# apirrone/Open_Duck_Playground

Measured on AMD Instinct MI355X. Metric: env-steps/sec open_duck_mini_v2 flat_terrain @8192 envs; 1/2/4/8-GPU scaling, higher is better.
Workload: dtype f32

## Files before the change

include/odk.h:

```cpp
#ifndef ODK_H
#define ODK_H

#include <stdint.h>

#ifdef __cplusplus
extern "C" {
#endif

typedef struct odk_model odk_model;
typedef struct odk_batch odk_batch;

enum odk_status {
  ODK_OK = 0,
  ODK_ERR_INVALID = -1,
  ODK_ERR_UNSUPPORTED = -2,
  ODK_ERR_HIP = -3,
  ODK_ERR_NOMEM = -4
};

#define ODK_NOBS 101
#define ODK_NPRIV 212
#define ODK_NOBS_STANDING 85
#define ODK_NPRIV_STANDING 153
#define ODK_ENV_JOYSTICK 0
// ... 348 lines not shown
} odk_step_tail;
int odk_adam_clip_packed_tail(float* params_dev, const float* grads_dev, float* m_dev, float* v_dev, float* acc_dev, long long n, float lr, float b1,
                              float b2, float eps, float max_grad_norm, float* fwd_packed_dev, long long n_fwd, float* bwd_packed_dev, long long n_bwd,
                              const odk_weight_table* table, int norm_blocks, const odk_step_tail* tail , void* stream);

#define ODK_GAE_HEAD_SAMPLES 32
typedef struct odk_gae_head_args {
  const float *logits, *values, *raw_action, *old_log_prob, *reward, *termination, *truncation, *noise;
  const long long* row_idx;
  const int* cursor;
  float *dlogits, *dvalues, *losses, *loss_partials, *adv_out, *vs_out, *stats_out;
  int B, T, action_size, n_traj, normalize_advantage;
  float gae_lambda, discount, clipping_epsilon, entropy_cost, grad_scale;
} odk_gae_head_args;
int odk_ppo_gae_head(const odk_gae_head_args* args, void* stream);

int odk_col_moments(const float* x_dev, long long rows, int w, int slices, double* partial_dev, void* stream);
int odk_moments_update(const double* partial_dev, int slices, int w, long long rows, double* count_dev, float* mean_dev, float* summed_variance_dev,
                       float* std_dev, float std_min, float std_max, void* stream);

int odk_colsum_fold(const float* const* partial_dev, float* const* colsum_dev, const int* widths, const int* nblk, int count, void* stream);

int odk_gather_rows(const float* const* src_dev, float* const* dst_dev, const int* row_floats, const long long* direct_base, int nfields,
                    const long long* idx_dev, int nrows, long long src_rows, void* stream);

int odk_batch_timing(odk_batch* b, int enable, float* avg_ms, int* launches);

#ifdef __cplusplus
}
#endif
// ... 2 lines not shown
```

open_duck_playground_amd/csrc/odk_learner.hip:

```cpp
#include <hip/hip_runtime.h>
#include <algorithm>
#include <utility>
#include <vector>
#include <stdint.h>
#include <string.h>

#include <type_traits>

#include "../../include/odk.h"
#include "odk_host.h"
#include "odk_poison.h"

int odk_func_lds_attr_(const void* fn, int slot, int bytes);

namespace {

__device__ __forceinline__ float wave_sum(float v) {
#pragma unroll
  for (int o = 32; o >= 1; o >>= 1) v += __shfl_xor(v, o);
  return v;
}
__device__ __forceinline__ float row16_sum(float v) {
#pragma unroll
  for (int o = 8; o >= 1; o >>= 1) v += __shfl_xor(v, o);
  return v;
}
__device__ float block_sum(float v, float* sh) {
  v = wave_sum(v);
  const int w = threadIdx.x >> 6, nw = blockDim.x >> 6;
  __syncthreads();
  if ((threadIdx.x & 63) == 0) sh[w] = v;
  __syncthreads();
  float t = 0.0f;
  for (int i = 0; i < nw; i++) t += sh[i];
  return t;
}
__device__ __forceinline__ float softplus(float x) { return x > 20.0f ? x : log1pf(__expf(x)); }
__device__ __forceinline__ float sigmoid(float x) { return 1.0f / (1.0f + __expf(-x)); }

__device__ __forceinline__ float gae_step(float r, float v, float mask, float nt, float discount, float lambda_, float& acc, float& v_next, float& vs_next,
                                          float& vs_t) {
  const float dn = __fmul_rn(discount, nt);
  const float delta = __fmul_rn(__fsub_rn(__fmaf_rn(dn, v_next, r), v), mask);
  acc = __fmaf_rn(__fmul_rn(__fmul_rn(dn, mask), lambda_), acc, delta);
  vs_t = __fadd_rn(acc, v);
  const float a = __fmul_rn(__fsub_rn(__fmaf_rn(dn, vs_next, r), v), mask);
  v_next = v; vs_next = vs_t;
  return a;
}

__global__ void gae_kernel(const float* __restrict__ trunc, const float* __restrict__ term, const float* __restrict__ rew,
                           const float* __restrict__ val, const float* __restrict__ boot, float* __restrict__ vs,
                           float* __restrict__ adv, float* __restrict__ stats, int B, int T, float lambda_, float discount) {
  __shared__ float sh[16];
#ifdef ODK_POISON_LDS
  odk_poison_fill(sh, sizeof(sh) / 4);
  __syncthreads();
#endif
  float s = 0.0f;
  for (int b = threadIdx.x; b < B; b += blockDim.x) {
    const size_t o = (size_t)b * T;
    float acc = 0.0f, v_next = boot[b], vs_next = boot[b];
    for (int t = T - 1; t >= 0; t--) {
// ... 85 lines not shown
      s = __fadd_rn(s, a);
    }
  }
  __syncthreads();
  for (int i = threadIdx.x; i < N; i += blockDim.x) { adv[i] = s_r[i]; vs[i] = s_v[i]; }
  if (!stats) return;
  const float n = (float)B * (float)T;
  const float mean = block_sum(s, sh) / n;
  float q = 0.0f;
  for (int b = threadIdx.x; b < B; b += blockDim.x)
    for (int t = 0; t < T; t++) { const float d = s_r[b * T + t] - mean; q = __fmaf_rn(d, d, q); }
  const float var = block_sum(q, sh) / n;
  if (threadIdx.x == 0) { stats[0] = mean; stats[1] = 1.0f / (sqrtf(var) + 1e-8f); }
}

struct HeadOut { float dloc, dscale_raw, dbaseline, lp, lv, le; };
__device__ __forceinline__ HeadOut head_sample(bool on, float loc, float raw, float a, float z, float advn, float old_lp, float vs_s, float base_s, float inv_n,
                                               float eps, float entropy_cost, float grad_scale) {
  const float HALF_LOG_2PI = 0.91893853320467274f, LOG2 = 0.69314718055994531f;
  const float scale = softplus(raw) + 0.001f, inv_scale = 1.0f / scale, lscale = __logf(scale);
  const float u = (a - loc) * inv_scale;
  const float ldj_a = 2.0f * (LOG2 - a - softplus(-2.0f * a));
  const float lp_j = on ? (-0.5f * u * u - lscale - HALF_LOG_2PI - ldj_a) : 0.0f;
  const float x = loc + scale * z;
  const float ldj_x = 2.0f * (LOG2 - x - softplus(-2.0f * x));
  const float ent_j = on ? (0.5f + HALF_LOG_2PI + lscale + ldj_x) : 0.0f;
  const float logp = row16_sum(lp_j), ent = row16_sum(ent_j);
  const float rho = __expf(logp - old_lp);
  const float rc = fminf(fmaxf(rho, 1.0f - eps), 1.0f + eps);
  const float s1 = rho * advn, s2 = rc * advn;
  const bool inside = rho >= 1.0f - eps && rho <= 1.0f + eps;
  const float dmin_drho = (inside || s1 < s2) ? advn : 0.0f;
  const float dL_dlogp = -dmin_drho * rho * inv_n;
  const float verr = vs_s - base_s;
  const float th = tanhf(x);
  const float ce = -entropy_cost * inv_n;
  HeadOut o;
  o.dloc = grad_scale * (dL_dlogp * u * inv_scale + ce * (-2.0f * th));
  o.dscale_raw = grad_scale * (dL_dlogp * (u * u - 1.0f) * inv_scale + ce * (inv_scale - 2.0f * th * z)) * sigmoid(raw);
  o.dbaseline = grad_scale * (-0.5f * verr * inv_n);
  o.lp = -fminf(s1, s2) * inv_n; o.lv = 0.25f * verr * verr * inv_n; o.le = -entropy_cost * ent * inv_n;
  return o;
}

__global__ void ppo_head_kernel(const float* __restrict__ logits, const float* __restrict__ raw_action, const float* __restrict__ old_logp,
                                const float* __restrict__ adv, const float* __restrict__ stats, const float* __restrict__ vs,
                                const float* __restrict__ baseline, const float* __restrict__ noise, float* __restrict__ dlogits,
                                float* __restrict__ dbaseline, float* __restrict__ losses, int n, int A, float eps, float entropy_cost,
                                float grad_scale) {
  const int lane = threadIdx.x & 15;
  const int s = (blockIdx.x * blockDim.x + threadIdx.x) >> 4;
  const bool live = s < n, on = live && lane < A;
  const int sc = live ? s : n - 1;
  float loc = 0.f, raw = 0.f, a = 0.f, z = 0.f;
  if (on) { loc = logits[(size_t)sc * 2 * A + lane]; raw = logits[(size_t)sc * 2 * A + A + lane]; a = raw_action[(size_t)sc * A + lane]; z = noise[(size_t)sc * A + lane]; }
  float advn = adv[sc];
  if (stats) advn = (advn - stats[0]) * stats[1];
  const HeadOut h = head_sample(on, loc, raw, a, z, advn, old_logp[sc], vs[sc], baseline[sc], 1.0f / (float)n, eps, entropy_cost, grad_scale);
// ... 768 lines not shown
```

open_duck_playground_amd/csrc/odk_mlp.hip:

```cpp
#include <hip/hip_runtime.h>
#include <stdint.h>
#include <stdlib.h>
#include <string.h>

#include "../../include/odk.h"
#include "odk_host.h"
#include "odk_poison.h"

namespace {

typedef float f32x4 __attribute__((ext_vector_type(4)));

constexpr int H1 = ODK_MLP_H1, H2 = ODK_MLP_H2, H3 = ODK_MLP_H3;
constexpr int TM = ODK_MLP_TILE;
constexpr int CH = 128;
constexpr int KIN_MAX = ODK_MLP_MAX_IN, NOUT_MAX = 32;
constexpr int PC = CH + 4, P2 = H2 + 4, P3 = H3 + 4, P4 = NOUT_MAX + 4;
constexpr int PX_MAX = KIN_MAX + 4;
constexpr int SLACK = 64;
static_assert(TM == 16 && KIN_MAX % 16 == 0, "tile = one 16-row MFMA block, padded input width");
constexpr int F_X = 0, F_C = F_X + TM * PX_MAX, F_H2 = F_C + TM * PC, F_TOTAL = F_H2 + TM * P2 + SLACK;
static_assert(TM * P3 <= TM * PX_MAX, "layer-3 output must fit in the X region");
static_assert(3 * 2 * 4 * 64 <= TM * PC, "output-layer partial blocks must fit in the chunk region");
static_assert(F_TOTAL * 4 <= 40 * 1024, "four forward workgroups per CU");
constexpr int B_D4 = 0, B_D3 = B_D4 + TM * P4, B_D2 = B_D3 + TM * P3, B_TOTAL = B_D2 + TM * P2 + SLACK;

__host__ __device__ constexpr int pad16(int k) { return (k + 15) & ~15; }

struct Net {
  const float* x; const float* in_mean; const float* in_std; const float* wf[4]; const float* wb[4]; const float* b[4];
  float* h[3]; float* g[3]; float* out; float* xp;
  const float* dout; float* dz[3]; float* doutp; float* bias_partial[4];
  int n, n_in, n_out, tile0;
  const long long* row_idx; const int* cursor; const float* x_tail; int traj_len, n_main, n_traj;
};
struct Map { int R, rounds, rem, vin2, pin2, v3, costly, on; };
struct Args { Net net[2]; int nnets; long long* prof; long long* wgprof; Map map; };
__device__ __forceinline__ void map_block(const Args& a, int b, int& net, int& tile) {
  const Map& m = a.map;
  if (!m.on) { net = (a.nnets > 1 && b >= a.net[1].tile0) ? 1 : 0; tile = b - a.net[net].tile0; return; }
  const int k = b % m.R, r = b / m.R;
  bool costly; int idx;
  if (k >= m.rem) { const int s2 = (k - m.rem) * m.rounds + r; costly = s2 < m.vin2; idx = costly ? s2 : s2 - m.vin2; }
  else { const int c = r * m.rem + k; costly = c < m.v3; idx = costly ? m.vin2 + c : m.pin2 + (c - m.v3); }
  net = costly ? m.costly : 1 - m.costly; tile = idx;
}
#define ODK_WG_BEGIN() long long wg_t0 = 0, wg_c0 = 0; if (a.wgprof) { wg_t0 = wall_clock64(); wg_c0 = clock64(); }
#define ODK_WG_END() do { if (a.wgprof && threadIdx.x == 0) { long long* o = a.wgprof + 4 * blockIdx.x; o[0] = wg_t0; o[1] = wall_clock64(); \
    o[2] = (long long)(unsigned)__builtin_amdgcn_s_getreg((31 << 11) | 4) | ((long long)(__builtin_amdgcn_s_getreg((31 << 11) | 20) & 0xF) << 32) | ((long long)net_i << 40); \
    o[3] = clock64() - wg_c0; } } while (0)
#define ODK_STAMP(i) do { if (a.prof && blockIdx.x == 0 && threadIdx.x == 0) a.prof[i] = clock64(); } while (0)

// ... 64 lines not shown
    for (int t = 0; t < 4; t++) {
      const int row = 4 * q + t;
      const float z = acc[k][t] + bias[k];
      const float sg = __builtin_amdgcn_rcpf(1.0f + __expf(-z));
      const float h = z * sg;
      Ls[row * P + 16 * k] = h;
      const bool live = row < rows_valid;
      hv[t] = live ? h : 0.0f;
      gv[t] = live ? sg + (h - h * sg) : 0.0f;
    }
    if (hq) {
      *reinterpret_cast<f32x4*>(hq + 64 * k) = hv;
      *reinterpret_cast<f32x4*>(gq + 64 * k) = gv;
    }
  }
}

__global__ void __launch_bounds__(256, MLP_WG_PER_CU) mlp_fwd_kernel(Args a) {
  extern __shared__ __attribute__((aligned(16))) float lds[];
#ifdef ODK_POISON_LDS
  odk_poison_fill(lds, F_TOTAL);
  __syncthreads();
#endif
  int net_i, tile;
  map_block(a, blockIdx.x, net_i, tile);
  const Net& N = a.net[net_i];
  const int m0 = tile * TM;
  const int rows_valid = N.n - m0;
  const int lane = threadIdx.x & 63, w = threadIdx.x >> 6, q = lane >> 4, c = lane & 15;
  const int kin = N.n_in, k16 = pad16(kin), PX = k16 + 4;
// ... 43 lines not shown
      for (int t = 0; t < T; t++) { const int k = lane + 64 * t; mu[t] = N.in_mean[k < kin ? k : 0]; sd[t] = N.in_std[k < kin ? k : 0]; }
#pragma unroll
      for (int i = 0; i < TM / 4; i++)
#pragma unroll
        for (int t = 0; t < T; t++) xv[i][t] = (xv[i][t] - mu[t]) / sd[t];
    }
    ODK_PIN();
#pragma unroll
    for (int i = 0; i < TM / 4; i++)
#pragma unroll
      for (int t = 0; t < T; t++) { const int k = lane + 64 * t; if (k < k16) X[(w + 4 * i) * PX + k] = k < kin ? xv[i][t] : 0.0f; }
  }
  __syncthreads();
  ODK_STAMP(1);
  const bool store = N.h[0] != nullptr;
  const size_t q0 = (size_t)(m0 >> 2);
  if (store) {
    for (int k = threadIdx.x; k < kin; k += 256)
#pragma unroll
      for (int qq = 0; qq < TM / 4; qq++) {
        f32x4 v;
#pragma unroll
        for (int t = 0; t < 4; t++) v[t] = X[(4 * qq + t) * PX + k];
        *reinterpret_cast<f32x4*>(N.xp + ((q0 + qq) * kin + k) * 4) = v;
      }
  }
  const size_t ql = q0 + q;
  f32x4 acc2[4];
  zero(acc2);
#pragma unroll
// ... 44 lines not shown
    float* R = C1;
    if (w > 0) {
#pragma unroll
      for (int k = 0; k < 2; k++)
#pragma unroll
        for (int t = 0; t < 4; t++) R[((w - 1) * 8 + 4 * k + t) * 64 + lane] = acc4[k][t];
    }
    __syncthreads();
    if (w == 0) {
#pragma unroll
      for (int k = 0; k < 2; k++)
#pragma unroll
        for (int t = 0; t < 4; t++) {
          const int row = 4 * q + t, e = 4 * k + t;
          const float z = ((acc4[k][t] + R[e * 64 + lane]) + (R[(8 + e) * 64 + lane] + R[(16 + e) * 64 + lane])) + bias4[k];
          if (16 * k + c < nout && row < rows_valid) N.out[(size_t)(m0 + row) * nout + 16 * k + c] = z;
        }
    }
  }
  ODK_STAMP(28);
  ODK_WG_END();
}

template <int NBLK>
__device__ __forceinline__ void load_g(f32x4 (&gv)[NBLK], const float* __restrict__ gq) {
#pragma unroll
  for (int k = 0; k < NBLK; k++) gv[k] = *reinterpret_cast<const f32x4*>(gq + 64 * k);
  ODK_PIN();
}
template <int NBLK>
__device__ __forceinline__ void bwd_epilogue(const f32x4 (&acc)[NBLK], const f32x4 (&gv)[NBLK], float* dzq, float* Ls, int P, float* partial, int q) {
#pragma unroll
  for (int k = 0; k < NBLK; k++) {
    f32x4 dv;
    float s = 0.0f;
#pragma unroll
    for (int t = 0; t < 4; t++) {
      const float dz = acc[k][t] * gv[k][t];
      dv[t] = dz;
      if (Ls) Ls[(4 * q + t) * P + 16 * k] = dz;
      s += dz;
    }
    *reinterpret_cast<f32x4*>(dzq + 64 * k) = dv;
    s += __shfl_xor(s, 16);
    s += __shfl_xor(s, 32);
    if (q == 0) partial[16 * k] = s;
  }
}

__global__ void __launch_bounds__(256, MLP_WG_PER_CU) mlp_bwd_kernel(Args a) {
  extern __shared__ __attribute__((aligned(16))) float lds[];
#ifdef ODK_POISON_LDS
  odk_poison_fill(lds, B_TOTAL);
  __syncthreads();
#endif
  int net_i, tile;
  map_block(a, blockIdx.x, net_i, tile);
  const Net& N = a.net[net_i];
  const int m0 = tile * TM;
  const int rows_valid = N.n - m0;
  const int lane = threadIdx.x & 63, w = threadIdx.x >> 6, q = lane >> 4, c = lane & 15;
  const int nout = N.n_out;
  float* D4 = lds + B_D4; float* D3 = lds + B_D3; float* D2 = lds + B_D2;
  Phase<2, 2> p3;
  Phase<4, 1> p2;
  Phase<8, 1> p1;
  ODK_WG_BEGIN();
  p3.prefetch(N.wb[3], H3, w * 32 + c, q, 0, pad16(nout) >> 4);
  for (int e = threadIdx.x; e < TM * NOUT_MAX; e += 256) {
    const int rr = e >> 5, k = e & 31;
    D4[rr * P4 + k] = (rr < rows_valid && k < nout) ? N.dout[(size_t)(m0 + rr) * nout + k] : 0.0f;
  }
  __syncthreads();
  const size_t q0 = (size_t)(m0 >> 2), ql = q0 + q;
  if (threadIdx.x < nout) {
    float s = 0.0f;
    for (int rr = 0; rr < TM; rr++) s += D4[rr * P4 + threadIdx.x];
    N.bias_partial[3][(size_t)tile * nout + threadIdx.x] = s;
  }
  for (int e = threadIdx.x; e < (TM / 4) * nout; e += 256) {
    const int qq = e / nout, k = e - qq * nout;
    f32x4 v;
#pragma unroll
    for (int t = 0; t < 4; t++) v[t] = D4[(4 * qq + t) * P4 + k];
    *reinterpret_cast<f32x4*>(N.doutp + ((q0 + qq) * nout + k) * 4) = v;
  }
  f32x4 gv3[2], gv2[4], gv1[8];
// ... 37 lines not shown
      const unsigned e = (unsigned)(i - t.off[k]);
      if (e < (unsigned)(t.rows[k] * t.cols[k])) {
        const unsigned o = e / (unsigned)t.cols[k], in = e - o * (unsigned)t.cols[k];
        pf[t.fwd[k] + ((in >> 2) * t.rows[k] + o) * 4 + (in & 3)] = v;
        if (t.bwd[k] >= 0) pb[t.bwd[k] + ((o >> 2) * t.cols[k] + in) * 4 + (o & 3)] = v;
        return;
      }
    }
  }
}

__global__ void pack_weights_kernel(const float* __restrict__ p, float* __restrict__ pf, float* __restrict__ pb, long long n, WeightTable t) {
  for (long long i = (long long)blockIdx.x * blockDim.x + threadIdx.x; i < n; i += (long long)gridDim.x * blockDim.x) packed_store(t, (int)i, p[i], pf, pb);
}

__device__ __forceinline__ float wave_sum(float v) {
#pragma unroll
  for (int o = 32; o >= 1; o >>= 1) v += __shfl_xor(v, o);
  return v;
}
__device__ float block_sum(float v, float* sh) {
  v = wave_sum(v);
  const int w = threadIdx.x >> 6, nw = blockDim.x >> 6;
  __syncthreads();
  if ((threadIdx.x & 63) == 0) sh[w] = v;
  __syncthreads();
  float t = 0.0f;
  for (int i = 0; i < nw; i++) t += sh[i];
  return t;
}
struct Tail { int* cursor; const float* partials; int npartials; float* losses; };
__device__ __forceinline__ void step_tail(const Tail& t) {
  if (t.cursor && blockIdx.x == 0 && threadIdx.x == 0) *t.cursor += 1;
  if (t.partials && blockIdx.x == gridDim.x - 1 && threadIdx.x < 64) {
    const int c = threadIdx.x & 3, q = threadIdx.x >> 2;
// ... 146 lines not shown
    a.out[f][c] = t;
  }
}

int check_launch(const char* what) {
  hipError_t e = hipGetLastError();
  if (e != hipSuccess) return odk_fail_(ODK_ERR_HIP, what);
  return ODK_OK;
}

long long* g_prof = nullptr;
long long* g_wgprof = nullptr;

int fill_args(Args& a, const odk_mlp_desc* nets, int count, bool backward, int& tiles, const char*& err) {
  a.nnets = count; tiles = 0; a.prof = backward ? nullptr : g_prof; a.wgprof = g_wgprof;
  for (int k = 0; k < 2; k++) {
    Net& N = a.net[k];
    if (k >= count) { N = a.net[0]; N.tile0 = 1 << 30; continue; }
    const odk_mlp_desc& d = nets[k];
    if (d.n <= 0 || d.n_in <= 0 || d.n_in > KIN_MAX || d.n_out <= 0 || d.n_out > NOUT_MAX) { err = "n_in must be 1..ODK_MLP_MAX_IN, n_out 1..32, n > 0"; return 1; }
    for (int l = 0; l < 4; l++) {
      const float* wp = backward ? d.wb[l] : d.wf[l];
      if ((!backward && (!d.b[l] || !wp)) || (backward && l > 0 && !wp)) { err = "missing packed weights / biases"; return 1; }
      if (((uintptr_t)wp & 15) != 0) { err = "packed weights must be 16-byte aligned"; return 1; }
    }
    const bool has_act = d.h[0] && d.h[1] && d.h[2] && d.g[0] && d.g[1] && d.g[2] && d.xp;
    if (!backward) {
      if (!d.x || !d.out) { err = "missing x / out"; return 1; }
      if ((d.in_mean != nullptr) != (d.in_std != nullptr)) { err = "in_mean / in_std: both or none"; return 1; }
      if (!has_act && (d.h[0] || d.h[1] || d.h[2] || d.g[0] || d.g[1] || d.g[2] || d.xp)) { err = "xp / h / g buffers: all seven or none"; return 1; }
// ... 56 lines not shown
  std::lock_guard<std::mutex> lock(mu);
  if (done[slot][dev]) return 0;
  if (hipFuncSetAttribute(fn, hipFuncAttributeMaxDynamicSharedMemorySize, bytes) != hipSuccess) return 1;
  done[slot][dev] = true;
  return 0;
}

extern "C" void odk_mlp_set_profile(long long* stamps_dev) { g_prof = stamps_dev; }
extern "C" void odk_mlp_set_wg_profile(long long* dev) { g_wgprof = dev; }

extern "C" int odk_mlp_forward(const odk_mlp_desc* nets, int count, void* stream) {
  if (!nets || count < 1 || count > 2) return odk_fail_(ODK_ERR_INVALID, "odk_mlp_forward: 1 or 2 networks");
  Args a; int tiles; const char* err = nullptr;
  if (fill_args(a, nets, count, false, tiles, err)) return odk_fail_(ODK_ERR_INVALID, err);
  const int fwd_lds = F_TOTAL * 4;
  if (odk_func_lds_attr_((const void*)mlp_fwd_kernel, 1, fwd_lds)) return odk_fail_(ODK_ERR_HIP, "odk_mlp_forward: the device refuses the kernel's dynamic LDS size");
  hipLaunchKernelGGL(mlp_fwd_kernel, dim3(tiles), dim3(256), fwd_lds, (hipStream_t)stream, a);
  return check_launch("odk_mlp_forward: launch failed");
}

extern "C" int odk_mlp_backward(const odk_mlp_desc* nets, int count, void* stream) {
  if (!nets || count < 1 || count > 2) return odk_fail_(ODK_ERR_INVALID, "odk_mlp_backward: 1 or 2 networks");
  Args a; int tiles; const char* err = nullptr;
  if (fill_args(a, nets, count, true, tiles, err)) return odk_fail_(ODK_ERR_INVALID, err);
  if (odk_func_lds_attr_((const void*)mlp_bwd_kernel, 2, B_TOTAL * 4)) return odk_fail_(ODK_ERR_HIP, "odk_mlp_backward: the device refuses the kernel's dynamic LDS size");
  hipLaunchKernelGGL(mlp_bwd_kernel, dim3(tiles), dim3(256), B_TOTAL * 4, (hipStream_t)stream, a);
  return check_launch("odk_mlp_backward: launch failed");
}

extern "C" int odk_pack_weights(const float* params_dev, long long n, float* fwd_packed_dev, long long n_fwd, float* bwd_packed_dev, long long n_bwd,
                                const odk_weight_table* table, void* stream) {
  WeightTable t;
  if (!params_dev || !fwd_packed_dev || !bwd_packed_dev || n <= 0 || fill_table(t, table, n, n_fwd, n_bwd))
// ... 76 lines not shown
```

open_duck_playground_amd/engine.py:

```python
from __future__ import annotations

import contextlib
import ctypes as C
import os
import re
import subprocess
from typing import Dict, List, Optional

import numpy as np

from .model import Model, asset_path

_CSRC = os.path.join(os.path.dirname(os.path.abspath(__file__)), "csrc")
LIB_PATH = os.environ.get("ODK_LIB", os.path.join(_CSRC, "libodk.so"))
POISON_LIB_PATH = os.path.join(_CSRC, "libodk_poison.so")


class OdkError(RuntimeError):
    pass


class OdkValueError(OdkError, ValueError):
    """An argument refused before any launch (`check_action_delays`): an OdkError that `except ValueError` catches too."""

# ... 228 lines not shown
        "odk_policy_sample": (I, [P, P, P, P, P, I, I, P]),
        "odk_adam_clip": (I, adam + [P]),
        "odk_silu_bwd_colsum": (I, [P, P, P, P, P, I, I, P]),
        "odk_colsum_partial": (I, [P, P, I, I, P]),
        "odk_colsum_finalize": (I, [PP, PP, IP, I, I, P]),
        "odk_dw_gemm": (I, [PP, PP, IP, IP, LP, I, IP, I, P, LL, P, C.POINTER(GradFinish), P]),
        "odk_mlp_forward": (I, [C.POINTER(MlpDesc), I, P]),
        "odk_mlp_backward": (I, [C.POINTER(MlpDesc), I, P]),
        "odk_dw_set_profile": (None, [P]),
        "odk_mlp_set_profile": (None, [P]),
        "odk_mlp_set_wg_profile": (None, [P]),
        "odk_pack_weights": (I, [P, LL, P, LL, P, LL, TABLE, P]),
        "odk_adam_clip_packed": (I, packed + [P]),
        "odk_adam_clip_packed_tail": (I, packed + [C.POINTER(StepTail), P]),
        "odk_ppo_gae_head": (I, [C.POINTER(GaeHeadArgs), P]),
        "odk_col_moments": (I, [P, LL, I, I, P, P]),
        "odk_moments_update": (I, [P, I, I, LL, P, P, P, P, F, F, P]),
        "odk_colsum_fold": (I, [PP, PP, IP, IP, I, P]),
        "odk_gather_rows": (I, [PP, PP, IP, LP, I, P, I, LL, P]),
        "odk_batch_timing": (I, [P, I, FP, IP]),
    }


SIGNATURES = _signatures()
EXPORTED_SYMBOLS = tuple(SIGNATURES)


def _check_placement(name: str, t, dtype, device: int) -> None:
    if t.dtype != dtype:
        raise OdkError(f"{name}: dtype must be {dtype}, got {t.dtype}")
# ... 483 lines not shown
            raise OdkError("GaeHead: the noise pool needs one [n, A] slot per schedule step")
        if n > 5120 or B > 1024:
            raise OdkError("GaeHead: B * T <= 5120, B <= 1024")
        a = GaeHeadArgs()
        a.logits, a.values, a.noise, a.dlogits, a.dvalues, a.losses = (t.data_ptr() for t in (logits, values, noise, dlogits, dvalues, losses))
        a.raw_action, a.old_log_prob, a.reward, a.termination, a.truncation = (rollout[k].data_ptr() for k in ("raw_action", "log_prob", "reward", "termination", "truncation"))
        a.row_idx, a.cursor = schedule.data_ptr(), cursor.data_ptr()
        a.adv_out, a.vs_out, a.stats_out, a.loss_partials = (None if t is None else t.data_ptr() for t in (adv, vs, stats, loss_partials))
        a.B, a.T, a.action_size, a.n_traj, a.normalize_advantage = int(B), int(T), int(A), n_traj, int(bool(cfg["normalize_advantage"]))
        a.gae_lambda, a.discount, a.clipping_epsilon, a.entropy_cost, a.grad_scale = (float(cfg["gae_lambda"]), float(cfg["discounting"]), float(cfg["clipping_epsilon"]),
                                                                                       float(cfg["entropy_cost"]), float(grad_scale))
        self.a, self.keep = a, (fl, rollout, schedule, cursor, adv, vs, stats, loss_partials)

    def __call__(self):
        _chk(load_library().odk_ppo_gae_head(C.byref(self.a), _stream(self.keep[0][0])))


class ColsumFold:

    def __init__(self, pairs, nblk):
        k = len(pairs)
        self.k, self.keep = k, pairs
        nblk = [int(nblk)] * k if isinstance(nblk, int) else [int(b) for b in nblk]
        for (p_, o_), nb in zip(pairs, nblk):
            _f32c(p_, o_)
            if p_.numel() < nb * o_.numel():
                raise OdkError("ColsumFold: partial buffer too small")
        self.nblk = (C.c_int * k)(*nblk)
        self.partial = (C.c_void_p * k)(*[p_.data_ptr() for p_, _ in pairs])
        self.out = (C.c_void_p * k)(*[o_.data_ptr() for _, o_ in pairs])
# ... 535 lines not shown
```

open_duck_playground_amd/ppo/learner.py:

```python
from __future__ import annotations

import os
import weakref
import tempfile
from functools import partial
from typing import Dict

import torch
import torch.nn.functional as F

from .. import engine
from .networks import PPONetworks

_DEBUG_NONFINITE = os.environ.get("ODK_DEBUG_NONFINITE") == "1"


_TUNED_ASSET = os.path.join(os.path.dirname(os.path.dirname(os.path.abspath(__file__))), "assets", "tunableop_gfx950.csv")


_scratch_files = []
_reported_validators = False


def _cleanup_tunableop():
# ... 250 lines not shown
        self.sample_noise = True
        self._gpool, self._pool_k = None, 0
        if use_graph:
            self._capture()

    def _bind_indexed(self):
        B, T, n, r = self.B, self.T, self.B * self.T, self.roll
        rows = dict(row_idx=self.sched, cursor=self.cursor, traj_len=T, n_main=n, n_traj=self.cap)
        self.policy.bind(r["obs"].view(self.cap * T, -1), self.dlogits, True, n, rows)
        self.value.bind(r["priv"].view(self.cap * T, -1), self.dval_all, True, n + B, dict(rows, x_tail=r["last_priv"]))
        self._build_fused()
        self.gae_head = engine.GaeHead(self.policy.zs[-1], self.value.zs[-1].view(-1), r, self._pool, self.sched, self.cursor, self.dlogits,
                                       self.dval_all.view(-1), self.losses, B, T, self.cfg, 1.0 / self.world, adv=self.adv.view(-1),
                                       vs=self.vs.view(-1), stats=self.stats, loss_partials=self.loss_partials)
        self._launches = [self.fused.forward, self.gae_head, self.fused.backward, self.dw_all]

    def _build_fused(self):
        dev = self.flat_p.device
        kslices = 8
        if getattr(self, "dw_ws", None) is None:
            self.dw_ws = torch.empty(kslices * engine.DwGemm.workspace_stride(self._n_par), device=dev)
        nets = (self.policy, self.value)
        self.wtable = engine.WeightTable([(o, w.shape[0], w.shape[1], l > 0) for f in nets for l, (o, w) in enumerate(zip(f.goff, f.W))])
        if getattr(self, "packed_f", None) is None:
            self.packed_f, self.packed_b = torch.zeros(self.wtable.fwd_size, device=dev), torch.zeros(self.wtable.bwd_size, device=dev)
        self.fused = engine.FusedMLP([f.fused_desc(self.wtable, 4 * k, self.packed_f, self.packed_b) for k, f in enumerate(nets)])
        self.dw_all = engine.DwGemm([l for f in nets for l in f.dw_layers], self.flat_g, self.dw_ws, kslices,
                                    bias=[(t, f.gb[i], f.tiles) for f in nets for i, t in enumerate(f.tile_sums)],
                                    acc=None if (self.split_update or not self._fused_norm) else self.acc)

# ... 291 lines not shown
```

Measured before the change: 21.12 million.

## Fold GAE into MLP forward and PPO head into MLP backward kernels

Moves the GAE computation into the tail of the fused MLP forward kernel: value tiles publish their outputs with atomic stores, and a ticket counter lets the last value tile run the GAE and advantage statistics in LDS. The PPO head (log-prob, clipping, entropy gradients, loss partials) is computed at the front of the backward kernel, so the separate gae_head launch is removed. This cuts one kernel launch and a round trip of intermediate data per update. In exchange, the forward kernel needs a much larger LDS allocation, which can lower occupancy, and the GAE work is serialised inside a single workgroup.

```diff
diff --git a/include/odk.h b/include/odk.h
--- a/include/odk.h
+++ b/include/odk.h
@@ -386,6 +386,8 @@
   float gae_lambda, discount, clipping_epsilon, entropy_cost, grad_scale;
 } odk_gae_head_args;
 int odk_ppo_gae_head(const odk_gae_head_args* args, void* stream);
+int odk_mlp_forward_gae(const odk_mlp_desc* nets, int count, const odk_gae_head_args* args, unsigned int* work_dev, void* stream);
+int odk_mlp_backward_head(const odk_mlp_desc* nets, int count, const odk_gae_head_args* args, const unsigned int* work_dev, void* stream);
 
 int odk_col_moments(const float* x_dev, long long rows, int w, int slices, double* partial_dev, void* stream);
 int odk_moments_update(const double* partial_dev, int slices, int w, long long rows, double* count_dev, float* mean_dev, float* summed_variance_dev,
diff --git a/open_duck_playground_amd/csrc/odk_learner.hip b/open_duck_playground_amd/csrc/odk_learner.hip
--- a/open_duck_playground_amd/csrc/odk_learner.hip
+++ b/open_duck_playground_amd/csrc/odk_learner.hip
@@ -10,6 +10,7 @@
 #include "../../include/odk.h"
 #include "odk_host.h"
 #include "odk_poison.h"
+#include "odk_ppo_head.h"
 
 int odk_func_lds_attr_(const void* fn, int slot, int bytes);
 
@@ -18,11 +19,6 @@
 __device__ __forceinline__ float wave_sum(float v) {
 #pragma unroll
   for (int o = 32; o >= 1; o >>= 1) v += __shfl_xor(v, o);
-  return v;
-}
-__device__ __forceinline__ float row16_sum(float v) {
-#pragma unroll
-  for (int o = 8; o >= 1; o >>= 1) v += __shfl_xor(v, o);
   return v;
 }
 __device__ float block_sum(float v, float* sh) {
@@ -34,19 +30,6 @@
   float t = 0.0f;
   for (int i = 0; i < nw; i++) t += sh[i];
   return t;
-}
-__device__ __forceinline__ float softplus(float x) { return x > 20.0f ? x : log1pf(__expf(x)); }
-__device__ __forceinline__ float sigmoid(float x) { return 1.0f / (1.0f + __expf(-x)); }
-
-__device__ __forceinline__ float gae_step(float r, float v, float mask, float nt, float discount, float lambda_, float& acc, float& v_next, float& vs_next,
-                                          float& vs_t) {
-  const float dn = __fmul_rn(discount, nt);
-  const float delta = __fmul_rn(__fsub_rn(__fmaf_rn(dn, v_next, r), v), mask);
-  acc = __fmaf_rn(__fmul_rn(__fmul_rn(dn, mask), lambda_), acc, delta);
-  vs_t = __fadd_rn(acc, v);
-  const float a = __fmul_rn(__fsub_rn(__fmaf_rn(dn, vs_next, r), v), mask);
-  v_next = v; vs_next = vs_t;
-  return a;
 }
 
 __global__ void gae_kernel(const float* __restrict__ trunc, const float* __restrict__ term, const float* __restrict__ rew,
@@ -162,34 +145,6 @@
   if (threadIdx.x == 0) { stats[0] = mean; stats[1] = 1.0f / (sqrtf(var) + 1e-8f); }
 }
 
-struct HeadOut { float dloc, dscale_raw, dbaseline, lp, lv, le; };
-__device__ __forceinline__ HeadOut head_sample(bool on, float loc, float raw, float a, float z, float advn, float old_lp, float vs_s, float base_s, float inv_n,
-                                               float eps, float entropy_cost, float grad_scale) {
-  const float HALF_LOG_2PI = 0.91893853320467274f, LOG2 = 0.69314718055994531f;
-  const float scale = softplus(raw) + 0.001f, inv_scale = 1.0f / scale, lscale = __logf(scale);
-  const float u = (a - loc) * inv_scale;
-  const float ldj_a = 2.0f * (LOG2 - a - softplus(-2.0f * a));
-  const float lp_j = on ? (-0.5f * u * u - lscale - HALF_LOG_2PI - ldj_a) : 0.0f;
-  const float x = loc + scale * z;
-  const float ldj_x = 2.0f * (LOG2 - x - softplus(-2.0f * x));
-  const float ent_j = on ? (0.5f + HALF_LOG_2PI + lscale + ldj_x) : 0.0f;
-  const float logp = row16_sum(lp_j), ent = row16_sum(ent_j);
-  const float rho = __expf(logp - old_lp);
-  const float rc = fminf(fmaxf(rho, 1.0f - eps), 1.0f + eps);
-  const float s1 = rho * advn, s2 = rc * advn;
-  const bool inside = rho >= 1.0f - eps && rho <= 1.0f + eps;
-  const float dmin_drho = (inside || s1 < s2) ? advn : 0.0f;
-  const float dL_dlogp = -dmin_drho * rho * inv_n;
-  const float verr = vs_s - base_s;
-  const float th = tanhf(x);
-  const float ce = -entropy_cost * inv_n;
-  HeadOut o;
-  o.dloc = grad_scale * (dL_dlogp * u * inv_scale + ce * (-2.0f * th));
-  o.dscale_raw = grad_scale * (dL_dlogp * (u * u - 1.0f) * inv_scale + ce * (inv_scale - 2.0f * th * z)) * sigmoid(raw);
-  o.dbaseline = grad_scale * (-0.5f * verr * inv_n);
-  o.lp = -fminf(s1, s2) * inv_n; o.lv = 0.25f * verr * verr * inv_n; o.le = -entropy_cost * ent * inv_n;
-  return o;
-}
 
 __global__ void ppo_head_kernel(const float* __restrict__ logits, const float* __restrict__ raw_action, const float* __restrict__ old_logp,
                                 const float* __restrict__ adv, const float* __restrict__ stats, const float* __restrict__ vs,
diff --git a/open_duck_playground_amd/csrc/odk_mlp.hip b/open_duck_playground_amd/csrc/odk_mlp.hip
--- a/open_duck_playground_amd/csrc/odk_mlp.hip
+++ b/open_duck_playground_amd/csrc/odk_mlp.hip
@@ -6,6 +6,7 @@
 #include "../../include/odk.h"
 #include "odk_host.h"
 #include "odk_poison.h"
+#include "odk_ppo_head.h"
 
 namespace {
 
@@ -35,7 +36,16 @@
   const long long* row_idx; const int* cursor; const float* x_tail; int traj_len, n_main, n_traj;
 };
 struct Map { int R, rounds, rem, vin2, pin2, v3, costly, on; };
-struct Args { Net net[2]; int nnets; long long* prof; long long* wgprof; Map map; };
+struct GaeTail {
+  unsigned* ticket; float *gr, *gf, *gold, *ga, *gn; const float *values, *reward, *term, *trunc, *raw_action, *old_logp, *noise; int A; const long long* idx; const int* cursor; float *adv, *vs, *stats;
+  int on, vnet, vtiles, B, T, n_traj; float lambda_, discount;
+};
+struct HeadFront {
+  const float *logits, *values, *gold, *ga, *gn, *adv, *vs, *stats;
+  float *dlogits, *dvalues, *loss_partials; int on, pnet, B, T, A, n_traj, normalize; float eps, entropy_cost, grad_scale;
+};
+static_assert(ODK_GAE_HEAD_SAMPLES == 2 * TM, "a loss partial = two tiles");
+struct Args { Net net[2]; int nnets; long long* prof; long long* wgprof; Map map; GaeTail gae; HeadFront head; };
 __device__ __forceinline__ void map_block(const Args& a, int b, int& net, int& tile) {
   const Map& m = a.map;
   if (!m.on) { net = (a.nnets > 1 && b >= a.net[1].tile0) ? 1 : 0; tile = b - a.net[net].tile0; return; }
@@ -130,6 +140,118 @@
       *reinterpret_cast<f32x4*>(gq + 64 * k) = gv;
     }
   }
+}
+
+__device__ __forceinline__ float wave_sum(float v) {
+#pragma unroll
+  for (int o = 32; o >= 1; o >>= 1) v += __shfl_xor(v, o);
+  return v;
+}
+
+__host__ __device__ constexpr int gae_lds_floats(int N) { return 2 * N + ((N + 3) >> 2) + 16 + 4; }
+constexpr int WORK_HEAD = 16;
+constexpr int GAE_MAX_ROWS = 5120, GAE_MAX_TRAJ = 1024;
+constexpr int FWD_LDS_CAP = (gae_lds_floats(GAE_MAX_ROWS) > F_TOTAL ? gae_lds_floats(GAE_MAX_ROWS) : F_TOTAL) * 4;
+
+__device__ __forceinline__ void gae_tail(const GaeTail& g, float* lds, int m0) {
+  const int B = g.B, T = g.T, N = B * T;
+  const long long* idx = g.idx + (size_t)(g.cursor ? *g.cursor : 0) * B;
+  const float nanv = __builtin_nanf("");
+  {
+    const int i = m0 + (int)(threadIdx.x >> 4), hl = threadIdx.x & 15, A = g.A;
+    if (i < N) {
+      const int b = i / T;
+      const long long jl = idx[b];
+      const bool ok = jl >= 0 && jl < g.n_traj;
+      const size_t o = (size_t)(ok ? jl : 0) * T + (i - b * T);
+      if (hl < A) {
+        const float act = g.raw_action[o * A + hl], z = g.noise[((size_t)(g.cursor ? *g.cursor : 0) * N + i) * A + hl];
+        g.ga[(size_t)i * A + hl] = ok ? act : nanv; g.gn[(size_t)i * A + hl] = z;
+      }
+      if (hl == 0) {
+        const float r = g.reward[o], tr = g.trunc[o], te = g.term[o], lp = g.old_logp[o];
+        __hip_atomic_store(g.gr + i, ok ? r : nanv, __ATOMIC_RELAXED, __HIP_MEMORY_SCOPE_AGENT);
+        __hip_atomic_store(g.gf + i, (tr != 0.0f ? 1.0f : 0.0f) + (te != 0.0f ? 2.0f : 0.0f), __ATOMIC_RELAXED, __HIP_MEMORY_SCOPE_AGENT);
+        g.gold[i] = ok ? lp : nanv;
+      }
+    }
+  }
+  float* s_r = lds; float* s_v = lds + N;
+  unsigned char* s_f = reinterpret_cast<unsigned char*>(lds + 2 * N);
+  float* sh = lds + 2 * N + ((N + 3) >> 2);
+  int* s_last = reinterpret_cast<int*>(sh + 16);
+  asm volatile("s_waitcnt vmcnt(0)" ::: "memory");
+  __syncthreads();
+  if (threadIdx.x == 0) *s_last = __hip_atomic_fetch_add(g.ticket, 1u, __ATOMIC_RELAXED, __HIP_MEMORY_SCOPE_AGENT) == (unsigned)(g.vtiles - 1) ? 1 : 0;
+  __syncthreads();
+  if (!*s_last) return;
+  if (threadIdx.x == 0) __hip_atomic_store(g.ticket, 0u, __ATOMIC_RELAXED, __HIP_MEMORY_SCOPE_AGENT);
+  __builtin_amdgcn_fence(__ATOMIC_ACQUIRE, "agent");
+  asm volatile("s_waitcnt vmcnt(0)" ::: "memory");
+  __syncthreads();
+  const int lane = threadIdx.x & 63, w = threadIdx.x >> 6;
+  constexpr int SB = 10;
+  for (int i0 = threadIdx.x; i0 < N; i0 += 256 * SB) {
+    float vv[SB], rr[SB], ff[SB];
+#pragma unroll
+    for (int u = 0; u < SB; u++) {
+      const int i = i0 + 256 * u < N ? i0 + 256 * u : N - 1;
+      vv[u] = __hip_atomic_load(g.values + i, __ATOMIC_RELAXED, __HIP_MEMORY_SCOPE_AGENT);
+      rr[u] = __hip_atomic_load(g.gr + i, __ATOMIC_RELAXED, __HIP_MEMORY_SCOPE_AGENT);
+      ff[u] = __hip_atomic_load(g.gf + i, __ATOMIC_RELAXED, __HIP_MEMORY_SCOPE_AGENT);
+    }
+    ODK_PIN();
+#pragma unroll
+    for (int u = 0; u < SB; u++) {
+      const int i = i0 + 256 * u;
+      if (i < N) { s_r[i] = rr[u]; s_v[i] = vv[u]; s_f[i] = (unsigned char)ff[u]; }
+    }
+  }
+  __syncthreads();
+  float s[2] = {0.0f, 0.0f};
+#pragma unroll
+  for (int kk = 0; kk < GAE_MAX_TRAJ / 256; kk++) {
+    const int b = threadIdx.x + 256 * kk;
+    if (b < B) {
+      const int o = b * T;
+      float acc = 0.0f, v_next = __hip_atomic_load(g.values + N + b, __ATOMIC_RELAXED, __HIP_MEMORY_SCOPE_AGENT), vs_next = v_next;
+#pragma unroll 4
+      for (int t = T - 1; t >= 0; t--) {
+        const int f = s_f[o + t];
+        const float te = (f & 2) ? 1.0f : 0.0f, tr = (f & 1) ? 1.0f : 0.0f;
+        const float mask = 1.0f - tr, nt = 1.0f - te, v = s_v[o + t], r = s_r[o + t];
+        float vs_t;
+        const float ad = gae_step(r, v, mask, nt, g.discount, g.lambda_, acc, v_next, vs_next, vs_t);
+        s_r[o + t] = ad;
+        s_v[o + t] = vs_t;
+        s[kk & 1] = __fadd_rn(s[kk & 1], ad);
+      }
+    }
+  }
+  auto sum512 = [&](float x0, float x1) -> float {
+    x0 = wave_sum(x0); x1 = wave_sum(x1);
+    __syncthreads();
+    if (lane == 0) { sh[w] = x0; sh[w + 4] = x1; }
+    __syncthreads();
+    float t = 0.0f;
+    for (int i = 0; i < 8; i++) t += sh[i];
+    return t;
+  };
+  const float n = (float)B * (float)T;
+  const float mean = sum512(s[0], s[1]) / n;
+  float q[2] = {0.0f, 0.0f};
+#pragma unroll
+  for (int kk = 0; kk < GAE_MAX_TRAJ / 256; kk++) {
+    const int b = threadIdx.x + 256 * kk;
+    if (b < B) {
+#pragma unroll 4
+      for (int t = 0; t < T; t++) { const float d = s_r[b * T + t] - mean; q[kk & 1] = __fmaf_rn(d, d, q[kk & 1]); }
+    }
+  }
+  const float var = sum512(q[0], q[1]) / n;
+  const float rstd = 1.0f / (sqrtf(var) + 1e-8f);
+  for (int i = threadIdx.x; i < N; i += 256) { g.adv[i] = s_r[i]; g.vs[i] = s_v[i]; }
+  if (threadIdx.x == 0) { g.stats[0] = mean; g.stats[1] = rstd; }
 }
 
 __global__ void __launch_bounds__(256, MLP_WG_PER_CU) mlp_fwd_kernel(Args a) {
@@ -203,6 +325,8 @@
   __syncthreads();
   ODK_STAMP(1);
   const bool store = N.h[0] != nullptr;
+  const bool publish = a.gae.on && net_i == a.gae.vnet;
+  if (publish) __builtin_amdgcn_s_setprio(3);
   const size_t q0 = (size_t)(m0 >> 2);
   if (store) {
     for (int k = threadIdx.x; k < kin; k += 256)
@@ -277,12 +401,16 @@
         for (int t = 0; t < 4; t++) {
           const int row = 4 * q + t, e = 4 * k + t;
           const float z = ((acc4[k][t] + R[e * 64 + lane]) + (R[(8 + e) * 64 + lane] + R[(16 + e) * 64 + lane])) + bias4[k];
-          if (16 * k + c < nout && row < rows_valid) N.out[(size_t)(m0 + row) * nout + 16 * k + c] = z;
+          if (16 * k + c < nout && row < rows_valid) {
+            float* o = N.out + (size_t)(m0 + row) * nout + 16 * k + c;
+            if (publish) __hip_atomic_store(o, z, __ATOMIC_RELAXED, __HIP_MEMORY_SCOPE_AGENT); else *o = z;
+          }
         }
     }
   }
   ODK_STAMP(28);
   ODK_WG_END();
+  if (publish) gae_tail(a.gae, lds, m0);
 }
 
 template <int NBLK>
@@ -308,6 +436,56 @@
     s += __shfl_xor(s, 16);
     s += __shfl_xor(s, 32);
     if (q == 0) partial[16 * k] = s;
+  }
+}
+
+__device__ __forceinline__ void head_front(const HeadFront& h, int net_i, int tile, int m0, float* D4, float* sh3) {
+  for (int e = threadIdx.x; e < TM * NOUT_MAX; e += 256) D4[(e >> 5) * P4 + (e & 31)] = 0.0f;
+  __syncthreads();
+  const int T = h.T, Nn = h.B * T, A = h.A;
+  const float n = (float)h.B * (float)T;
+  if (net_i != h.pnet) {
+    const int row = m0 + (int)threadIdx.x;
+    if (threadIdx.x < TM && row < Nn) {
+      const float d = head_dbaseline(h.vs[row], h.values[row], 1.0f / n, h.grad_scale);
+      D4[threadIdx.x * P4] = d;
+      h.dvalues[row] = d;
+    }
+    return;
+  }
+  const float mean = h.stats[0], rstd = h.stats[1];
+  const int lane = threadIdx.x & 15, rr = threadIdx.x >> 4, w = threadIdx.x >> 6;
+  const int npass = (tile & 1) ? 1 : 2;
+  for (int p = 0; p < npass; p++) {
+    const int smp = m0 + TM * p + rr;
+    const bool live = smp < Nn, on = live && lane < A;
+    const int sc = live ? smp : Nn - 1;
+    float loc = 0.f, raw = 0.f, act = 0.f, z = 0.f;
+    if (on) { loc = h.logits[(size_t)sc * 2 * A + lane]; raw = h.logits[(size_t)sc * 2 * A + A + lane]; act = h.ga[(size_t)sc * A + lane]; z = h.gn[(size_t)sc * A + lane]; }
+    const float old_lp = h.gold[sc], base_s = h.values[sc];
+    float advn = h.adv[sc];
+    if (h.normalize) advn = (advn - mean) * rstd;
+    const HeadOut o = head_sample(on, loc, raw, act, z, advn, old_lp, h.vs[sc], base_s, 1.0f / n, h.eps, h.entropy_cost, h.grad_scale);
+    if (p == 0 && on) {
+      D4[rr * P4 + lane] = o.dloc; D4[rr * P4 + A + lane] = o.dscale_raw;
+      h.dlogits[(size_t)smp * 2 * A + lane] = o.dloc;
+      h.dlogits[(size_t)smp * 2 * A + A + lane] = o.dscale_raw;
+    }
+    if (npass == 2) {
+      float lp = 0.f, lv = 0.f, le = 0.f;
+      if (live && lane == 0) { lp = o.lp; lv = o.lv; le = o.le; }
+      lp = wave_sum(lp); lv = wave_sum(lv); le = wave_sum(le);
+      if ((threadIdx.x & 63) == 0) { sh3[4 * p + w] = lp; sh3[8 + 4 * p + w] = lv; sh3[16 + 4 * p + w] = le; }
+    }
+  }
+  if (npass == 2) {
+    __syncthreads();
+    if (threadIdx.x == 0) {
+      float tx = 0.0f, ty = 0.0f, tz = 0.0f;
+      for (int i = 0; i < 8; i++) { tx += sh3[i]; ty += sh3[8 + i]; tz += sh3[16 + i]; }
+      float* o = h.loss_partials + 4 * (tile >> 1);
+      o[0] = tx + ty + tz; o[1] = tx; o[2] = ty; o[3] = tz;
+    }
   }
 }
 
@@ -330,10 +508,12 @@
   Phase<8, 1> p1;
   ODK_WG_BEGIN();
   p3.prefetch(N.wb[3], H3, w * 32 + c, q, 0, pad16(nout) >> 4);
-  for (int e = threadIdx.x; e < TM * NOUT_MAX; e += 256) {
-    const int rr = e >> 5, k = e & 31;
-    D4[rr * P4 + k] = (rr < rows_valid && k < nout) ? N.dout[(size_t)(m0 + rr) * nout + k] : 0.0f;
-  }
+  if (a.head.on) head_front(a.head, net_i, tile, m0, D4, D3);
+  else
+    for (int e = threadIdx.x; e < TM * NOUT_MAX; e += 256) {
+      const int rr = e >> 5, k = e & 31;
+      D4[rr * P4 + k] = (rr < rows_valid && k < nout) ? N.dout[(size_t)(m0 + rr) * nout + k] : 0.0f;
+    }
   __syncthreads();
   const size_t q0 = (size_t)(m0 >> 2), ql = q0 + q;
   if (threadIdx.x < nout) {
@@ -401,11 +581,6 @@
   for (long long i = (long long)blockIdx.x * blockDim.x + threadIdx.x; i < n; i += (long long)gridDim.x * blockDim.x) packed_store(t, (int)i, p[i], pf, pb);
 }
 
-__device__ __forceinline__ float wave_sum(float v) {
-#pragma unroll
-  for (int o = 32; o >= 1; o >>= 1) v += __shfl_xor(v, o);
-  return v;
-}
 __device__ float block_sum(float v, float* sh) {
   v = wave_sum(v);
   const int w = threadIdx.x >> 6, nw = blockDim.x >> 6;
@@ -582,6 +757,7 @@
 
 int fill_args(Args& a, const odk_mlp_desc* nets, int count, bool backward, int& tiles, const char*& err) {
   a.nnets = count; tiles = 0; a.prof = backward ? nullptr : g_prof; a.wgprof = g_wgprof;
+  memset(&a.gae, 0, sizeof(a.gae)); memset(&a.head, 0, sizeof(a.head));
   for (int k = 0; k < 2; k++) {
     Net& N = a.net[k];
     if (k >= count) { N = a.net[0]; N.tile0 = 1 << 30; continue; }
@@ -668,9 +844,55 @@
   Args a; int tiles; const char* err = nullptr;
   if (fill_args(a, nets, count, false, tiles, err)) return odk_fail_(ODK_ERR_INVALID, err);
   const int fwd_lds = F_TOTAL * 4;
-  if (odk_func_lds_attr_((const void*)mlp_fwd_kernel, 1, fwd_lds)) return odk_fail_(ODK_ERR_HIP, "odk_mlp_forward: the device refuses the kernel's dynamic LDS size");
+  if (odk_func_lds_attr_((const void*)mlp_fwd_kernel, 1, FWD_LDS_CAP)) return odk_fail_(ODK_ERR_HIP, "odk_mlp_forward: the device refuses the kernel's dynamic LDS size");
   hipLaunchKernelGGL(mlp_fwd_kernel, dim3(tiles), dim3(256), fwd_lds, (hipStream_t)stream, a);
   return check_launch("odk_mlp_forward: launch failed");
+}
+
+static const char* head_fold_check(const odk_mlp_desc* nets, int count, const odk_gae_head_args* g) {
+  if (!nets || count != 2 || !g) return "two networks (policy, value) and the head's arguments";
+  if (g->B <= 0 || g->T <= 0 || g->action_size <= 0 || g->action_size > 16 || g->n_traj <= 0) return "bad arguments (action_size must be 1..16)";
+  if ((long long)g->B * g->T > GAE_MAX_ROWS || g->B > GAE_MAX_TRAJ) return "B * T <= 5120 and B <= 1024";
+  const int n = g->B * g->T;
+  if (nets[0].n != n || nets[0].n_out != 2 * g->action_size || nets[1].n != n + g->B || nets[1].n_out != 1) return "nets[0]: B T rows x 2 A logits; nets[1]: B T + B rows x 1 value";
+  if (nets[0].out != g->logits || nets[1].out != g->values) return "logits / values must be the two networks' outputs";
+  if (!g->raw_action || !g->old_log_prob || !g->reward || !g->termination || !g->truncation || !g->noise || !g->row_idx || !g->dlogits || !g->dvalues ||
+      !g->loss_partials || !g->adv_out || !g->vs_out || !g->stats_out) return "missing pointers (adv_out, vs_out, stats_out and loss_partials are required here)";
+  return nullptr;
+}
+
+extern "C" int odk_mlp_forward_gae(const odk_mlp_desc* nets, int count, const odk_gae_head_args* g, unsigned int* work_dev, void* stream) {
+  if (const char* bad = head_fold_check(nets, count, g)) return odk_fail_(ODK_ERR_INVALID, bad);
+  if (!work_dev) return odk_fail_(ODK_ERR_INVALID, "odk_mlp_forward_gae: work_dev");
+  Args a; int tiles; const char* err = nullptr;
+  if (fill_args(a, nets, count, false, tiles, err)) return odk_fail_(ODK_ERR_INVALID, err);
+  GaeTail& t = a.gae;
+  const int n = g->B * g->T;
+  t.ticket = work_dev; t.gr = reinterpret_cast<float*>(work_dev) + WORK_HEAD; t.gf = t.gr + n; t.gold = t.gf + n; t.ga = t.gold + n; t.gn = t.ga + (size_t)n * g->action_size;
+  t.raw_action = g->raw_action; t.old_logp = g->old_log_prob; t.noise = g->noise; t.A = g->action_size; t.values = g->values; t.reward = g->reward; t.term = g->termination; t.trunc = g->truncation; t.idx = g->row_idx; t.cursor = g->cursor;
+  t.adv = g->adv_out; t.vs = g->vs_out; t.stats = g->stats_out; t.on = 1; t.vnet = 1; t.vtiles = tiles - a.net[1].tile0; t.B = g->B; t.T = g->T; t.n_traj = g->n_traj;
+  t.lambda_ = g->gae_lambda; t.discount = g->discount;
+  const int need = gae_lds_floats(g->B * g->T), fwd_lds = (need > F_TOTAL ? need : F_TOTAL) * 4;
+  if (odk_func_lds_attr_((const void*)mlp_fwd_kernel, 1, FWD_LDS_CAP)) return odk_fail_(ODK_ERR_HIP, "odk_mlp_forward_gae: the device refuses the kernel's dynamic LDS size");
+  hipLaunchKernelGGL(mlp_fwd_kernel, dim3(tiles), dim3(256), fwd_lds, (hipStream_t)stream, a);
+  return check_launch("odk_mlp_forward_gae: launch failed");
+}
+
+extern "C" int odk_mlp_backward_head(const odk_mlp_desc* nets, int count, const odk_gae_head_args* g, const unsigned int* work_dev, void* stream) {
+  if (const char* bad = head_fold_check(nets, count, g)) return odk_fail_(ODK_ERR_INVALID, bad);
+  if (!work_dev) return odk_fail_(ODK_ERR_INVALID, "odk_mlp_backward_head: work_dev");
+  Args a; int tiles; const char* err = nullptr;
+  if (fill_args(a, nets, count, true, tiles, err)) return odk_fail_(ODK_ERR_INVALID, err);
+  HeadFront& h = a.head;
+  h.logits = g->logits; h.values = g->values; h.adv = g->adv_out; h.vs = g->vs_out;
+  h.stats = g->stats_out; h.dlogits = g->dlogits; h.dvalues = g->dvalues; h.loss_partials = g->loss_partials;
+  const int n = g->B * g->T;
+  h.gold = reinterpret_cast<const float*>(work_dev) + WORK_HEAD + 2 * n; h.ga = h.gold + n; h.gn = h.ga + (size_t)n * g->action_size;
+  h.on = 1; h.pnet = 0; h.B = g->B; h.T = g->T; h.A = g->action_size; h.n_traj = g->n_traj; h.normalize = g->normalize_advantage;
+  h.eps = g->clipping_epsilon; h.entropy_cost = g->entropy_cost; h.grad_scale = g->grad_scale;
+  if (odk_func_lds_attr_((const void*)mlp_bwd_kernel, 2, B_TOTAL * 4)) return odk_fail_(ODK_ERR_HIP, "odk_mlp_backward_head: the device refuses the kernel's dynamic LDS size");
+  hipLaunchKernelGGL(mlp_bwd_kernel, dim3(tiles), dim3(256), B_TOTAL * 4, (hipStream_t)stream, a);
+  return check_launch("odk_mlp_backward_head: launch failed");
 }
 
 extern "C" int odk_mlp_backward(const odk_mlp_desc* nets, int count, void* stream) {
diff --git a/open_duck_playground_amd/csrc/odk_ppo_head.h b/open_duck_playground_amd/csrc/odk_ppo_head.h
--- /dev/null
+++ b/open_duck_playground_amd/csrc/odk_ppo_head.h
@@ -0,0 +1,59 @@
+#pragma once
+#include <hip/hip_runtime.h>
+
+namespace {
+
+__device__ __forceinline__ float row16_sum(float v) {
+#pragma unroll
+  for (int o = 8; o >= 1; o >>= 1) v += __shfl_xor(v, o);
+  return v;
+}
+__device__ __forceinline__ float softplus(float x) { return x > 20.0f ? x : log1pf(__expf(x)); }
+__device__ __forceinline__ float sigmoid(float x) { return 1.0f / (1.0f + __expf(-x)); }
+
+__device__ __forceinline__ float gae_step(float r, float v, float mask, float nt, float discount, float lambda_, float& acc, float& v_next, float& vs_next,
+                                          float& vs_t) {
+  const float dn = __fmul_rn(discount, nt);
+  const float delta = __fmul_rn(__fsub_rn(__fmaf_rn(dn, v_next, r), v), mask);
+  acc = __fmaf_rn(__fmul_rn(__fmul_rn(dn, mask), lambda_), acc, delta);
+  vs_t = __fadd_rn(acc, v);
+  const float a = __fmul_rn(__fsub_rn(__fmaf_rn(dn, vs_next, r), v), mask);
+  v_next = v; vs_next = vs_t;
+  return a;
+}
+
+__device__ __forceinline__ float head_dbaseline(float vs_s, float base_s, float inv_n, float grad_scale) {
+  const float verr = vs_s - base_s;
+  return grad_scale * (-0.5f * verr * inv_n);
+}
+
+struct HeadOut { float dloc, dscale_raw, dbaseline, lp, lv, le; };
+__device__ __forceinline__ HeadOut head_sample(bool on, float loc, float raw, float a, float z, float advn, float old_lp, float vs_s, float base_s, float inv_n,
+                                               float eps, float entropy_cost, float grad_scale) {
+  const float HALF_LOG_2PI = 0.91893853320467274f, LOG2 = 0.69314718055994531f;
+  const float scale = softplus(raw) + 0.001f, inv_scale = 1.0f / scale, lscale = __logf(scale);
+  const float u = (a - loc) * inv_scale;
+  const float ldj_a = 2.0f * (LOG2 - a - softplus(-2.0f * a));
+  const float lp_j = on ? (-0.5f * u * u - lscale - HALF_LOG_2PI - ldj_a) : 0.0f;
+  const float x = loc + scale * z;
+  const float ldj_x = 2.0f * (LOG2 - x - softplus(-2.0f * x));
+  const float ent_j = on ? (0.5f + HALF_LOG_2PI + lscale + ldj_x) : 0.0f;
+  const float logp = row16_sum(lp_j), ent = row16_sum(ent_j);
+  const float rho = __expf(logp - old_lp);
+  const float rc = fminf(fmaxf(rho, 1.0f - eps), 1.0f + eps);
+  const float s1 = rho * advn, s2 = rc * advn;
+  const bool inside = rho >= 1.0f - eps && rho <= 1.0f + eps;
+  const float dmin_drho = (inside || s1 < s2) ? advn : 0.0f;
+  const float dL_dlogp = -dmin_drho * rho * inv_n;
+  const float verr = vs_s - base_s;
+  const float th = tanhf(x);
+  const float ce = -entropy_cost * inv_n;
+  HeadOut o;
+  o.dloc = grad_scale * (dL_dlogp * u * inv_scale + ce * (-2.0f * th));
+  o.dscale_raw = grad_scale * (dL_dlogp * (u * u - 1.0f) * inv_scale + ce * (inv_scale - 2.0f * th * z)) * sigmoid(raw);
+  o.dbaseline = grad_scale * (-0.5f * verr * inv_n);
+  o.lp = -fminf(s1, s2) * inv_n; o.lv = 0.25f * verr * verr * inv_n; o.le = -entropy_cost * ent * inv_n;
+  return o;
+}
+
+}
diff --git a/open_duck_playground_amd/engine.py b/open_duck_playground_amd/engine.py
--- a/open_duck_playground_amd/engine.py
+++ b/open_duck_playground_amd/engine.py
@@ -266,6 +266,8 @@
         "odk_adam_clip_packed": (I, packed + [P]),
         "odk_adam_clip_packed_tail": (I, packed + [C.POINTER(StepTail), P]),
         "odk_ppo_gae_head": (I, [C.POINTER(GaeHeadArgs), P]),
+        "odk_mlp_forward_gae": (I, [C.POINTER(MlpDesc), I, C.POINTER(GaeHeadArgs), P, P]),
+        "odk_mlp_backward_head": (I, [C.POINTER(MlpDesc), I, C.POINTER(GaeHeadArgs), P, P]),
         "odk_col_moments": (I, [P, LL, I, I, P, P]),
         "odk_moments_update": (I, [P, I, I, LL, P, P, P, P, F, F, P]),
         "odk_colsum_fold": (I, [PP, PP, IP, IP, I, P]),
@@ -779,6 +781,28 @@
 
     def __call__(self):
         _chk(load_library().odk_ppo_gae_head(C.byref(self.a), _stream(self.keep[0][0])))
+
+
+class HeadFold:
+
+    WORK_HEAD = 16
+
+    def __init__(self, fused: "FusedMLP", head: "GaeHead"):
+        import torch
+        if fused.k != 2 or not all(fused.train):
+            raise OdkError("HeadFold: a training FusedMLP of (policy, value)")
+        a = head.a
+        if not (a.adv_out and a.vs_out and a.stats_out and a.loss_partials):
+            raise OdkError("HeadFold: the GaeHead needs adv, vs, stats and loss_partials")
+        self.fused, self.head = fused, head
+        self.work = torch.zeros(self.WORK_HEAD + (3 + 2 * a.action_size) * a.B * a.T, dtype=torch.int32, device=fused.keep[0]["x"].device)
+        self.ticket = self.work[:1]
+
+    def forward(self):
+        _chk(load_library().odk_mlp_forward_gae(self.fused.desc, 2, C.byref(self.head.a), self.work.data_ptr(), _stream(self.work)))
+
+    def backward(self):
+        _chk(load_library().odk_mlp_backward_head(self.fused.desc, 2, C.byref(self.head.a), self.work.data_ptr(), _stream(self.work)))
 
 
 class ColsumFold:
diff --git a/open_duck_playground_amd/ppo/learner.py b/open_duck_playground_amd/ppo/learner.py
--- a/open_duck_playground_amd/ppo/learner.py
+++ b/open_duck_playground_amd/ppo/learner.py
@@ -288,6 +288,10 @@
                                        self.dval_all.view(-1), self.losses, B, T, self.cfg, 1.0 / self.world, adv=self.adv.view(-1),
                                        vs=self.vs.view(-1), stats=self.stats, loss_partials=self.loss_partials)
         self._launches = [self.fused.forward, self.gae_head, self.fused.backward, self.dw_all]
+        self.head_fold = None
+        if not self.split_update:
+            self.head_fold = engine.HeadFold(self.fused, self.gae_head)
+            self._launches = [self.head_fold.forward, self.head_fold.backward, self.dw_all]
 
     def _build_fused(self):
         dev = self.flat_p.device
```

Measured after the change: 21.12 million. About the same (-0.0%).
